# HeewoongNoh/DOSTransformer

Hardware: NVIDIA B200
Metric: train-step crystals/sec (fwd+bwd) (higher is better)
Workload: dtype bf16x3 operands, f32 accumulate

## Files before the change

dostransformer_b200/_lib.py:

```python
from __future__ import annotations

import ctypes as C
import os
from typing import Optional

import torch

_HERE = os.path.dirname(os.path.abspath(__file__))
LIB_PATH = os.environ.get("DOST_B200_LIB") or os.path.join(_HERE, "libdost_b200.so")

F32, F64 = 0, 1
ACT_NONE, ACT_RELU, ACT_LEAKY, ACT_PRELU = 0, 1, 2, 3
KC, MC = 0, 1
PREC_FMA, PREC_BF16X3, PREC_BF16 = 0, 1, 2
PRECISIONS = {"fp32": PREC_FMA, "bf16x3": PREC_BF16X3, "bf16": PREC_BF16}

_lib: Optional[C.CDLL] = None
ABI_VERSION = 15
DEVERR_MESSAGES = {1: "an index (edge_index / batch / system) is outside its table",
                   2: "a crystal has more atoms than the padding length given by the host (max_num_nodes)"}


class Seg(C.Structure):
    _fields_ = [("base", C.c_void_p), ("ld", C.c_longlong), ("idx", C.c_void_p), ("div", C.c_int),
# ... 36 lines not shown
        ("res_bstride", C.c_longlong),
        ("b_rowoff", C.c_void_p), ("c_rowoff", C.c_void_p), ("c_rowlim", C.c_void_p),
        ("colsum", C.c_void_p),
        ("out_gate", C.c_void_p), ("dact_gate", C.c_void_p), ("ld_gate", C.c_longlong),
    ]


_SIGNATURES = {
    "dost_abi_version": (C.c_int, []),
    "dost_last_error": (C.c_char_p, []),
    "dost_launch_count": (C.c_longlong, []),
    "dost_reset_launch_count": (None, []),
    "dost_device_errors_init": (C.c_int, []),
    "dost_device_errors": (C.c_uint, [C.c_int]),
    "dost_imax_scalar": (C.c_int, [C.c_void_p, C.c_int, C.c_void_p]),
    "dost_cast_i64_i32": (C.c_int, [C.c_void_p, C.c_void_p, C.c_longlong, C.c_void_p]),
    "dost_csr_workspace_bytes": (C.c_size_t, [C.c_longlong, C.c_longlong]),
    "dost_csr_build": (C.c_int, [C.c_void_p, C.c_longlong, C.c_longlong, C.c_void_p, C.c_void_p, C.c_void_p,
                                 C.c_void_p, C.c_size_t, C.c_void_p]),
    "dost_gemm_workspace_bytes": (C.c_size_t, [C.POINTER(Gemm)]),
    "dost_gemm": (C.c_int, [C.POINTER(Gemm), C.c_void_p, C.c_size_t, C.c_void_p]),
    "dost_gemm_bf16_workspace_bytes": (C.c_size_t, [C.POINTER(GemmBf16)]),
    "dost_gemm_bf16": (C.c_int, [C.POINTER(GemmBf16), C.c_void_p, C.c_size_t, C.c_void_p]),
    "dost_split_planes": (C.c_int, [C.c_void_p, C.c_longlong, C.c_longlong, C.c_int, C.c_void_p, C.c_void_p, C.c_longlong,
                                    C.c_void_p]),
    "dost_split_planes_multi": (C.c_int, [C.c_int, C.c_void_p, C.c_void_p, C.c_void_p, C.c_void_p, C.c_void_p, C.c_void_p,
                                          C.c_void_p, C.c_void_p]),
    "dost_split_planes_colsum_workspace_bytes": (C.c_size_t, [C.c_longlong, C.c_int, C.c_longlong]),
    "dost_split_planes_colsum": (C.c_int, [C.c_void_p, C.c_longlong, C.c_longlong, C.c_int, C.c_void_p, C.c_void_p, C.c_longlong,
                                           C.c_void_p, C.c_void_p, C.c_size_t, C.c_void_p]),
    "dost_ln_fwd_planes": (C.c_int, [C.c_void_p, C.c_longlong, C.c_void_p, C.c_void_p, C.c_void_p, C.c_void_p, C.c_longlong,
                                     C.c_void_p, C.c_void_p, C.c_void_p, C.c_void_p,
                                     C.c_void_p, C.c_void_p, C.c_longlong, C.c_void_p, C.c_longlong, C.c_int, C.c_void_p]),
    "dost_ln_bwd_planes_workspace_bytes": (C.c_size_t, [C.c_longlong, C.c_int]),
    "dost_ln_bwd_planes": (C.c_int, [C.c_void_p, C.c_longlong, C.c_void_p, C.c_longlong, C.c_void_p, C.c_void_p, C.c_void_p,
                                     C.c_void_p, C.c_void_p, C.c_longlong, C.c_void_p, C.c_void_p, C.c_void_p, C.c_longlong,
                                     C.c_void_p, C.c_void_p, C.c_void_p, C.c_void_p, C.c_longlong, C.c_int, C.c_void_p,
                                     C.c_size_t, C.c_void_p]),
    "dost_rowdot_fwd": (C.c_int, [C.c_void_p, C.c_longlong, C.c_void_p, C.c_void_p, C.c_void_p, C.c_longlong, C.c_int, C.c_void_p]),
    "dost_rowdot_bwd_workspace_bytes": (C.c_size_t, [C.c_longlong, C.c_int]),
    "dost_rowdot_bwd": (C.c_int, [C.c_void_p, C.c_void_p, C.c_longlong, C.c_void_p, C.c_void_p, C.c_void_p, C.c_longlong, C.c_int,
                                  C.c_void_p, C.c_size_t, C.c_void_p]),
    "dost_colsum_planes_workspace_bytes": (C.c_size_t, [C.c_longlong, C.c_int]),
    "dost_colsum_planes": (C.c_int, [C.c_void_p, C.c_void_p, C.c_longlong, C.c_longlong, C.c_int, C.c_void_p, C.c_void_p,
                                     C.c_size_t, C.c_void_p]),
    "dost_ln_fwd": (C.c_int, [C.c_int, C.c_void_p, C.c_longlong, C.c_void_p, C.c_void_p, C.c_void_p, C.c_void_p,
# ... 196 lines not shown
```

dostransformer_b200/csrc/gemm_bf.cu:

```cuda
#include <cuda.h>
#include <cuda_bf16.h>
#include <cstdlib>
#include "common.cuh"
#include "tc_ptx.cuh"

namespace dost {
namespace bf {

constexpr int BM = 128, BK = 64;
constexpr int kMaxStages = 6;
constexpr int kEpiBytes = 8 * 4096;
constexpr int kSmemBudget = 225 * 1024;

struct Maps {
  CUtensorMap a_hi[3], a_lo[3], b_hi, b_lo;
  CUtensorMap b_hi2, b_lo2;
  CUtensorMap c_out, c_hi, c_lo;
  CUtensorMap c_pre;
};

struct Params {
  int M, N, K;
  int a_nseg, a_kend[3];
  int a_mc, b_mc;
  int zmode, kchunk;
  long long c_bstride, res_bstride;
  const int* b_rowoff;
  const int* c_rowoff;
  const int* c_rowlim;
  int m_tiles, n_tiles, total_tiles;
  const float* bias;
  const float* rowbias; long long ld_rowbias; int rowbias_div;
  int act; float act_slope; const float* prelu_slope;
  float* out_pre; long long ld_pre;
  const __nv_bfloat16* dact_hi; long long ld_dact; float dact_slope;
  const float* residual; long long ld_res;
  float* out; long long ldc; int accumulate;
  __nv_bfloat16* out_hi; __nv_bfloat16* out_lo; long long ld_op;
  float* ws;
  float* colpart;
  unsigned int* out_gate;
  const unsigned int* dact_gate;
  long long ld_gate;
  int tma_epi;
};
// ... 48 lines not shown
  asm volatile("cp.async.bulk.tensor.2d.global.shared::cta.bulk_group [%0, {%1, %2}], [%3];" ::"l"(map), "r"(c0), "r"(c1), "r"(src)
               : "memory");
}

struct TileInfo {
  int m0, n0, kbeg, kend, nkt, z;
};
template <int BN, bool CTA2>
__device__ __forceinline__ TileInfo tile_info(const Params& p, int tile, int rank) {
  TileInfo t;
  const int per_z = p.m_tiles * p.n_tiles;
  t.z = tile / per_z;
  const int rem = tile - t.z * per_z;
  const int mt = rem / p.n_tiles, nt = rem - mt * p.n_tiles;
  t.m0 = mt * (CTA2 ? 2 * BM : BM) + rank * BM;
  t.n0 = nt * BN;
  t.kbeg = 0;
  t.kend = p.K;
  if (p.zmode == 2) {
    t.kbeg = t.z * p.kchunk;
    t.kend = min(p.K, t.kbeg + p.kchunk);
  }
  t.nkt = (t.kend > t.kbeg) ? (t.kend - t.kbeg + BK - 1) / BK : 0;
  return t;
}

template <int NSPLIT, int BN, bool CTA2, int EW = 8>
__global__ void __launch_bounds__((EW + 2) * 32, 1) gemm_bf_kernel(const __grid_constant__ Maps maps, const Params p) {
  constexpr int kEpiWarps = EW;
  constexpr bool SPLIT = NSPLIT == 3;
  constexpr int BNL = CTA2 ? BN / 2 : BN;
  constexpr int A_BYTES = BM * BK * 2, B_BYTES = BNL * BK * 2;
  constexpr int STAGE_BYTES = (SPLIT ? 2 : 1) * (A_BYTES + B_BYTES);
  constexpr int NSTAGE_RAW = (kSmemBudget - kEpiBytes) / STAGE_BYTES;
  constexpr int NSTAGE = NSTAGE_RAW < kMaxStages ? NSTAGE_RAW : kMaxStages;
  static_assert(NSTAGE >= 2, "need at least two smem stages");

  extern __shared__ __align__(1024) unsigned char smem_raw[];
  unsigned char* smem = reinterpret_cast<unsigned char*>((reinterpret_cast<uintptr_t>(smem_raw) + 1023) & ~uintptr_t(1023));
  float* epi_smem = reinterpret_cast<float*>(smem + NSTAGE * STAGE_BYTES);
  __shared__ __align__(8) unsigned long long bars[2 * kMaxStages + 4];
  __shared__ uint32_t tmem_base_s;

  const int warp = threadIdx.x >> 5, lane = threadIdx.x & 31;
  const uint32_t full0 = smem_u32(&bars[0]), empty0 = smem_u32(&bars[kMaxStages]);
  const uint32_t accf0 = smem_u32(&bars[2 * kMaxStages]), acce0 = smem_u32(&bars[2 * kMaxStages + 2]);
// ... 18 lines not shown
                   : "memory");
      asm volatile("tcgen05.relinquish_alloc_permit.cta_group::2.sync.aligned;" ::: "memory");
    } else {
      asm volatile("tcgen05.alloc.cta_group::1.sync.aligned.shared::cta.b32 [%0], %1;" ::"r"(smem_u32(&tmem_base_s)), "r"(512)
                   : "memory");
      asm volatile("tcgen05.relinquish_alloc_permit.cta_group::1.sync.aligned;" ::: "memory");
    }
  }
  tc_fence_before();
  __syncthreads();
  if (CTA2) cluster_sync_all();
  tc_fence_after();
  const uint32_t tmem_base = tmem_base_s;
  const bool a_mc = p.a_mc != 0, b_mc = p.b_mc != 0;

  if (warp == kEpiWarps + 1) {
    if (lane == 0) {
      int stage = 0;
      uint32_t phase = 0;
      for (int tile = tile0; tile < p.total_tiles; tile += tile_step) {
        const TileInfo t = tile_info<BN, CTA2>(p, tile, rank);
        const int nb0 = t.n0 + rank * BNL;
        int seg = 0;
        for (int kt = 0; kt < t.nkt; ++kt) {
          const int k0 = t.kbeg + kt * BK;
          while (seg + 1 < p.a_nseg && k0 >= p.a_kend[seg]) ++seg;
          const int kseg = k0 - (seg == 0 ? 0 : p.a_kend[seg - 1]);
          mbar_wait(empty0 + 8 * stage, phase ^ 1);
          const uint32_t bar = CTA2 ? mapa_rank(full0 + 8 * stage, 0) : full0 + 8 * stage;
          if (!CTA2) mbar_expect_tx(bar, STAGE_BYTES);
          else if (rank == 0) mbar_expect_tx(full0 + 8 * stage, 2 * STAGE_BYTES);
          const uint32_t sA = smem_u32(smem + stage * STAGE_BYTES);
          const uint32_t sB = sA + (SPLIT ? 2 : 1) * A_BYTES;
          const int zb = (p.zmode == 1) ? t.z : 0;
          auto load = [&](uint32_t dst, const CUtensorMap* m, int c0, int c1, int c2) {
            if (CTA2) tma_load_3d_2cta(dst, m, c0, c1, c2, bar);
            else tma_load_3d(dst, m, c0, c1, c2, bar);
          };
          const int brow = p.b_rowoff ? __ldg(p.b_rowoff + t.z) : 0;
          const int zbb = p.b_rowoff ? 0 : zb;
          if (!a_mc) {
            load(sA, &maps.a_hi[seg], kseg, t.m0, zb);
            if (SPLIT) load(sA + A_BYTES, &maps.a_lo[seg], kseg, t.m0, zb);
          } else {
#pragma unroll
            for (int b = 0; b < BM / 64; ++b) {
              load(sA + b * 8192, &maps.a_hi[0], t.m0 + 64 * b, k0, zb);
              if (SPLIT) load(sA + A_BYTES + b * 8192, &maps.a_lo[0], t.m0 + 64 * b, k0, zb);
            }
          }
          if (!b_mc) {
            load(sB, CTA2 ? &maps.b_hi2 : &maps.b_hi, k0, nb0 + brow, zbb);
            if (SPLIT) load(sB + B_BYTES, CTA2 ? &maps.b_lo2 : &maps.b_lo, k0, nb0 + brow, zbb);
          } else {
#pragma unroll
            for (int b = 0; b < BNL / 64; ++b) {
              load(sB + b * 8192, &maps.b_hi, nb0 + 64 * b, k0 + brow, zbb);
              if (SPLIT) load(sB + B_BYTES + b * 8192, &maps.b_lo, nb0 + 64 * b, k0 + brow, zbb);
            }
          }
          if (++stage == NSTAGE) {
            stage = 0;
            phase ^= 1;
          }
        }
      }
    }
  } else if (warp == kEpiWarps) {
    const uint32_t idesc = make_idesc(CTA2 ? 2 * BM : BM, BN, a_mc, b_mc);
    const uint32_t a_kstep = a_mc ? (2048 >> 4) : (32 >> 4);
    const uint32_t b_kstep = b_mc ? (2048 >> 4) : (32 >> 4);
    int stage = 0;
    uint32_t phase = 0;
    uint32_t acc_phase[2] = {0, 0};
    int local = 0;
    for (int tile = tile0; tile < p.total_tiles && rank == 0; tile += tile_step, ++local) {
      const TileInfo t = tile_info<BN, CTA2>(p, tile, rank);
      const int buf = local & 1;
      mbar_wait(acce0 + 8 * buf, acc_phase[buf] ^ 1);
      tc_fence_after();
      const uint32_t tmem_d = tmem_base + buf * BN;
// ... 746 lines not shown
  attr[0].val.clusterDim.x = 2;
  attr[0].val.clusterDim.y = 1;
  attr[0].val.clusterDim.z = 1;
  cfg.attrs = attr;
  cfg.numAttrs = 1;
  cudaError_t e = cudaLaunchKernelEx(&cfg, kern, maps, p);
  if (e != cudaSuccess) {
    set_error("gemm_bf16: cluster launch failed: %s", cudaGetErrorString(e));
    return DOST_ERR_LAUNCH;
  }
  return check_launch("gemm_bf16 (CTA pairs)");
}

static bool use_cta_pairs(int M, int N) {
  static const int enabled = [] {
    const char* e = getenv("DOST_GEMM_2CTA");
    return (e && e[0] == '0') ? 0 : 1;
  }();
  return enabled && M > 128 && N > 128;
}

static inline bool al16(const void* ptr) { return (reinterpret_cast<uintptr_t>(ptr) & 15) == 0; }

static int run(const dost_gemm_bf16_t* h, void* workspace, size_t workspace_bytes, cudaStream_t st) {
  DOST_REQUIRE(h->M > 0 && h->N > 0 && h->K > 0, "gemm_bf16: bad shape M=%d N=%d K=%d", h->M, h->N, h->K);
  DOST_REQUIRE(h->precision == DOST_PREC_BF16X3 || h->precision == DOST_PREC_BF16, "gemm_bf16: precision must be bf16x3 or bf16");
  DOST_REQUIRE(h->N % 4 == 0, "gemm_bf16: N must be a multiple of 4 (got %d)", h->N);
  const bool split3 = h->precision == DOST_PREC_BF16X3;
  const bool a_mc = h->a_mode == DOST_MC, b_mc = h->b_mode == DOST_MC;
  const int nseg = a_mc ? 1 : h->a_nseg;
  DOST_REQUIRE(nseg >= 1 && nseg <= 3, "gemm_bf16: a_nseg must be 1..3");
  const int bn = h->N <= 64 ? 64 : (h->N <= 128 ? 128 : 256);
  const bool pairs = use_cta_pairs(h->M, h->N);
  const int batch = h->batch < 1 ? 1 : h->batch;
  DOST_REQUIRE(!(batch > 1 && h->split_k > 1), "gemm_bf16: batch and split_k are exclusive");
  DOST_REQUIRE(batch == 1 || (h->a_nseg <= 1 && !h->rowbias && !h->out_pre && !h->dact_hi && !h->out_hi),
               "gemm_bf16: batched problems support bias / activation / residual / fp32 stores only");
  DOST_REQUIRE(batch == 1 || (h->a_bstride % 8 == 0 && h->b_bstride % 8 == 0 && h->c_bstride % 4 == 0 && h->res_bstride % 4 == 0),
               "gemm_bf16: batch strides must keep 16-byte alignment");

  Maps maps;
  Params p;
  p.M = h->M; p.N = h->N; p.K = h->K;
  p.a_nseg = nseg;
  p.a_mc = a_mc; p.b_mc = b_mc;
  int kacc = 0;
  for (int s = 0; s < nseg; ++s) {
// ... 35 lines not shown
        if (rc == DOST_OK && split3) rc = make_map(&maps.b_lo, pl.lo, h->K, pl.rows, pl.ld, bn);
        if (rc == DOST_OK && pairs) rc = make_map(&maps.b_hi2, pl.hi, h->K, pl.rows, pl.ld, 128);
        if (rc == DOST_OK && pairs && split3) rc = make_map(&maps.b_lo2, pl.lo, h->K, pl.rows, pl.ld, 128);
      } else {
        rc = make_map(&maps.b_hi, pl.hi, h->N, pl.rows, pl.ld, 64);
        if (rc == DOST_OK && split3) rc = make_map(&maps.b_lo, pl.lo, h->N, pl.rows, pl.ld, 64);
      }
    } else if (!b_mc) {
      const long long nrows = (pl.rows > 0 && pl.rows < h->N) ? pl.rows : h->N;
      rc = make_map(&maps.b_hi, pl.hi, h->K, nrows, pl.ld, bn, batch, h->b_bstride);
      if (rc == DOST_OK && split3) rc = make_map(&maps.b_lo, pl.lo, h->K, nrows, pl.ld, bn, batch, h->b_bstride);
      if (rc == DOST_OK && pairs) rc = make_map(&maps.b_hi2, pl.hi, h->K, nrows, pl.ld, 128, batch, h->b_bstride);
      if (rc == DOST_OK && pairs && split3) rc = make_map(&maps.b_lo2, pl.lo, h->K, nrows, pl.ld, 128, batch, h->b_bstride);
    } else {
      rc = make_map(&maps.b_hi, pl.hi, h->N, h->K, pl.ld, 64, batch, h->b_bstride);
      if (rc == DOST_OK && split3) rc = make_map(&maps.b_lo, pl.lo, h->N, h->K, pl.ld, 64, batch, h->b_bstride);
    }
    if (rc != DOST_OK) return rc;
    if (!split3) maps.b_lo = maps.b_hi;
    if (!pairs || b_mc) maps.b_hi2 = maps.b_hi;
    if (!pairs || b_mc || !split3) maps.b_lo2 = maps.b_hi2;
  }
  const int split = h->split_k < 1 ? 1 : h->split_k;
  p.zmode = split > 1 ? 2 : (batch > 1 ? 1 : 0);
  p.c_bstride = h->c_bstride;
  p.res_bstride = h->res_bstride;
  p.b_rowoff = h->b_rowoff;
  p.c_rowoff = h->c_rowoff;
  p.c_rowlim = h->c_rowlim;
  DOST_REQUIRE(!p.c_rowoff || p.c_rowlim, "gemm_bf16: ragged output needs both c_rowoff and c_rowlim");
  DOST_REQUIRE(split == 1 || !(p.b_rowoff || p.c_rowoff || p.c_rowlim), "gemm_bf16: ragged problems cannot be split along K");
  p.kchunk = 0;
  p.ws = nullptr;
  if (split > 1) {
    DOST_REQUIRE(!h->bias && !h->rowbias && h->act == DOST_ACT_NONE && !h->out_pre && !h->dact_hi && !h->residual && !h->out_hi,
                 "gemm_bf16: split_k supports only plain (accumulating) fp32 stores");
    const size_t need = sizeof(float) * (size_t)split * h->M * h->N;
    if (!workspace || workspace_bytes < need) {
      set_error("gemm_bf16: split_k workspace too small (%zu < %zu)", workspace_bytes, need);
      return DOST_ERR_WORKSPACE;
    }
    int kchunk = (h->K + split - 1) / split;
    p.kchunk = ((kchunk + BK - 1) / BK) * BK;
    p.ws = (float*)workspace;
  }
  p.m_tiles = pairs ? (h->M + 2 * BM - 1) / (2 * BM) : (h->M + BM - 1) / BM;
// ... 86 lines not shown
  }
  if (split > 1) {
    const long long total4 = (long long)h->M * h->N / 4;
    int blocks = (int)min64((total4 + 255) / 256, (long long)kNumSMs * 8);
    if (blocks < 1) blocks = 1;
    splitk_reduce_kernel<<<blocks, 256, 0, st>>>(p.ws, h->out, h->ldc, h->M, h->N, split, h->accumulate);
    rc = check_launch("gemm_bf16 split-k reduce");
  }
  return rc;
}

}
}

extern "C" size_t dost_gemm_bf16_workspace_bytes(const dost_gemm_bf16_t* g) {
  if (!g) return 0;
  if (g->colsum) return sizeof(float) * ((size_t)((g->M + 31) / 32) + dost::bf::kMidRows) * g->N;
  if (g->split_k <= 1) return 0;
  return sizeof(float) * (size_t)g->split_k * g->M * g->N;
}

extern "C" int dost_gemm_bf16(const dost_gemm_bf16_t* g, void* workspace, size_t workspace_bytes, dost_stream_t stream) {
  DOST_REQUIRE(g != nullptr, "gemm_bf16: null descriptor");
  return dost::bf::run(g, workspace, workspace_bytes, (cudaStream_t)stream);
}

extern "C" size_t dost_split_planes_colsum_workspace_bytes(long long rows, int cols, long long ldp) {
  return sizeof(float) * (size_t)dost::bf::split_colsum_chunks(rows, (int)ldp) * cols;
}

extern "C" int dost_split_planes_colsum(const float* x, long long ld, long long rows, int cols, void* hi, void* lo, long long ldp,
                                        float* colsum, void* workspace, size_t workspace_bytes, dost_stream_t stream) {
  DOST_REQUIRE(x && hi && colsum, "split_planes_colsum: null pointer");
  DOST_REQUIRE(rows > 0 && cols > 0 && ldp >= cols && ldp % 8 == 0, "split_planes_colsum: need rows > 0, ldp %% 8 == 0, ldp >= cols");
  DOST_REQUIRE(((uintptr_t)hi & 15) == 0 && ((uintptr_t)lo & 15) == 0, "split_planes_colsum: planes must be 16-byte aligned");
  const int nch = dost::bf::split_colsum_chunks(rows, (int)ldp);
  const size_t need = sizeof(float) * (size_t)nch * cols;
  if (!workspace || workspace_bytes < need) {
    dost::set_error("split_planes_colsum: workspace too small (%zu < %zu)", workspace_bytes, need);
    return DOST_ERR_WORKSPACE;
  }
  const int vec_ok = (((uintptr_t)x & 15) == 0 && ld % 4 == 0) ? 1 : 0;
  const long long rpc = (rows + nch - 1) / nch;
  dim3 grid((unsigned)((ldp / 8 + 31) / 32), nch);
  cudaStream_t st = (cudaStream_t)stream;
  dost::bf::split_planes_colsum_kernel<<<grid, 256, 0, st>>>(x, ld, rows, cols, (__nv_bfloat16*)hi, (__nv_bfloat16*)lo, (int)ldp, vec_ok,
                                                             rpc, (float*)workspace);
// ... 55 lines not shown
```

dostransformer_b200/ops.py:

```python
from __future__ import annotations

import ctypes as C
import math
from contextlib import nullcontext
import os
from dataclasses import dataclass, field
from typing import List, Optional, Sequence, Tuple

import torch

from . import _lib as L

NUM_SMS = 148

_PRECISION = L.PREC_FMA


def set_precision(name: str) -> None:
    global _PRECISION
    _PRECISION = L.PRECISIONS[name]


def get_precision() -> int:
    return _PRECISION
# ... 361 lines not shown
        cache[_planes_key(w)] = ((base._version, base.data_ptr(), _PLANES_GENERATION), Planes(hi, lo, w.shape[0], w.shape[1]))


def _planes_c(pl: Planes, width: int) -> L.PlanesC:
    c = L.PlanesC()
    c.hi = pl.hi.data_ptr()
    c.lo = pl.lo.data_ptr() if pl.lo is not None else None
    c.ld = pl.ld
    c.rows = pl.rows
    c.width = width
    return c


def gemm_planes(*, M: int, N: int, K: int, a: Sequence[Planes], a_mode: int, b: Planes, b_mode: int,
                out: Optional[torch.Tensor] = None, bias: Optional[torch.Tensor] = None,
                rowbias: Optional[torch.Tensor] = None, rowbias_div: int = 1, act: int = L.ACT_NONE, act_slope: float = 0.0,
                prelu_slope: Optional[torch.Tensor] = None, out_pre: Optional[torch.Tensor] = None,
                dact: Optional[Planes] = None, dact_slope: float = 0.0, residual: Optional[torch.Tensor] = None,
                accumulate: bool = False, split_k: int = 1, out_planes: Optional[Planes] = None,
                ldc: Optional[int] = None, prec: Optional[int] = None, batch: int = 1, a_bstride: int = 0, b_bstride: int = 0,
                c_bstride: int = 0, res_bstride: int = 0, ld_res: Optional[int] = None, b_rows: Optional[int] = None,
                b_rowoff: Optional[torch.Tensor] = None, c_rowoff: Optional[torch.Tensor] = None,
                c_rowlim: Optional[torch.Tensor] = None, colsum_out: Optional[torch.Tensor] = None,
                out_gate: Optional[torch.Tensor] = None, dact_gate: Optional[torch.Tensor] = None) -> None:
    g = L.GemmBf16()
    g.M, g.N, g.K = M, N, K
    g.a_mode, g.a_nseg = a_mode, len(a)
    for i, pl in enumerate(a):
        g.a[i] = _planes_c(pl, pl.cols if a_mode == L.KC else K)
    g.b_mode = b_mode
    g.b = _planes_c(b, 0)
    g.b.rows = b_rows if b_rows is not None else 0
    g.bias = bias.data_ptr() if bias is not None else None
    if rowbias is not None:
        g.rowbias, g.ld_rowbias, g.rowbias_div = rowbias.data_ptr(), _ld(rowbias), rowbias_div
    g.act, g.act_slope = act, act_slope
    g.prelu_slope = prelu_slope.data_ptr() if prelu_slope is not None else None
    if out_pre is not None:
        g.out_pre, g.ld_pre = out_pre.data_ptr(), _ld(out_pre)
    if dact is not None:
        g.dact_hi, g.ld_dact, g.dact_slope = dact.hi.data_ptr(), dact.ld, dact_slope
    if residual is not None:
        g.residual, g.ld_res = residual.data_ptr(), (ld_res if ld_res is not None else _ld(residual))
    if out is not None:
        g.out = out.data_ptr()
        g.ldc = ldc if ldc is not None else _ld(out)
    g.accumulate = 1 if accumulate else 0
    g.batch, g.a_bstride, g.b_bstride, g.c_bstride, g.res_bstride = batch, a_bstride, b_bstride, c_bstride, res_bstride
    g.b_rowoff = b_rowoff.data_ptr() if b_rowoff is not None else None
    g.c_rowoff = c_rowoff.data_ptr() if c_rowoff is not None else None
    g.c_rowlim = c_rowlim.data_ptr() if c_rowlim is not None else None
    if out_planes is not None:
        g.out_hi = out_planes.hi.data_ptr()
        g.out_lo = out_planes.lo.data_ptr() if out_planes.lo is not None else None
        g.ld_op = out_planes.ld
    g.split_k = split_k
    g.precision = _PRECISION if prec is None else prec
    g.colsum = colsum_out.data_ptr() if colsum_out is not None else None
    if out_gate is not None:
        g.out_gate, g.ld_gate = out_gate.data_ptr(), out_gate.stride(0)
    if dact_gate is not None:
        g.dact_gate, g.ld_gate, g.dact_slope = dact_gate.data_ptr(), dact_gate.stride(0), dact_slope
    lib = L.lib()
    ws, nb = None, 0
    if split_k > 1 or colsum_out is not None:
        nb = lib.dost_gemm_bf16_workspace_bytes(C.byref(g))
        ws = _ws(nb, b.hi.device)
    L.check(lib.dost_gemm_bf16(C.byref(g), L.p(ws), nb, L.stream()), "gemm_bf16")


def gate_bits_ok(M: int, N: int) -> bool:
    return M >= 32 and N % 32 == 0 and os.environ.get("DOST_GEMM_TMA_EPI", "1") != "0" and not L.switch("DOST_NO_FFN_GATE")


def tc_active(t: torch.Tensor) -> bool:
    return _PRECISION != L.PREC_FMA and t.dtype == torch.float32


def _with_lo() -> bool:
    return _PRECISION != L.PREC_BF16


def ln_fwd_planes(x2d: torch.Tensor, gamma, beta, slope=None, *, want_y: bool = False, want_planes: bool = True,
                  gather_add=None):
    M, W = x2d.shape
    ga = ia = gb = ib = None
    ldg = 0
    if gather_add is not None:
        ga, ia, gb, ib = gather_add
        ldg = _ld(ga)
        assert _ld(gb) == ldg
# ... 877 lines not shown
            dop = _grad_planes(d_out, S * T, H)
            d_out = d_out.contiguous()
            dP = torch.empty(S * T, npad, dtype=torch.float32, device=dev)
            gemm_planes(M=T, N=npad, K=H, a=[dop], a_mode=L.KC, b=kvp, b_mode=L.KC, b_rows=N + B, out=dP, batch=S,
                        a_bstride=T * dop.ld, c_bstride=T * npad, b_rowoff=ptr_ext)
            dsp = empty_planes(S * T, npad, dev, _with_lo())
            if ctx.fused and ctx.drop_p > 0:
                scores = torch.empty(S * T, npad, dtype=torch.float32, device=dev)
                gemm_planes(M=T, N=npad, K=H, a=[qp], a_mode=L.KC, b=kvp, b_mode=L.KC, b_rows=N + B, out=scores, batch=S,
                            a_bstride=T * qp.ld, c_bstride=T * npad, b_rowoff=ptr_ext)
            if ctx.fused and ctx.drop_p == 0:
                _ds_from_planes(pp, dP, S * T, npad, float(H) ** -0.5, dsp)
            else:
                L.check(lib.dost_xattn_softmax_bwd_dseed(L.p(scores), L.p(lse), L.p(dP), L.p(g.ptr), L.p(g.nmax), S * T, B, T, npad,
                                                         float(H) ** -0.5, L.p(dsp.hi), L.p(dsp.lo), dsp.ld, ctx.drop_p, ctx.seed,
                                                         L.p(ctx.seed_offset), L.stream()), "xattn_softmax_bwd")
            dq = torch.empty(S, T, H, dtype=torch.float32, device=dev)
            gemm_planes(M=T, N=H, K=npad, a=[dsp], a_mode=L.KC, b=kvp, b_mode=L.MC, b_rows=N + B, out=dq.view(S * T, H), batch=S,
                        a_bstride=T * dsp.ld, c_bstride=T * H, b_rowoff=ptr_ext)
            dkv = torch.empty(N, H, dtype=torch.float32, device=dev)
            dbrows = torch.empty(B, H, dtype=torch.float32, device=dev)
            if not L.switch("DOST_NO_XATTN_PADDED_DK"):
                dpad = torch.empty(S * npad, H, dtype=torch.float32, device=dev)
                gemm_planes(M=npad, N=H, K=T, a=[dsp], a_mode=L.MC, b=qp, b_mode=L.MC, out=dpad, batch=S, a_bstride=T * dsp.ld,
                            b_bstride=T * qp.ld, c_bstride=npad * H)
                gemm_planes(M=npad, N=H, K=T, a=[pp], a_mode=L.MC, b=dop, b_mode=L.MC, out=dpad, accumulate=True, batch=S,
                            a_bstride=T * pp.ld, b_bstride=T * dop.ld, c_bstride=npad * H)
                L.check(lib.dost_xattn_kv_pad_split(L.p(dpad), npad, reps, L.p(g.batch), L.p(g.ptr), N, B, H, L.p(dkv), L.p(dbrows),
                                                    L.stream()), "xattn_kv_pad_split")
                dph = colsum(dbrows)
                d_q = colsum(dq.view(S, T * H)).view(T, H) if ctx.bcast_q else dq
                d_resid = colsum(d_out.view(S, T * H)).view(T, H) if ctx.bcast_r else d_out
                return d_q, dkv, dph, d_resid, None, None, None, None, None, None, None
            dext = torch.empty(N + B, H, dtype=torch.float32, device=dev)
            p1, n1 = g.ragged(1)
            for rep in range(reps):
                r0, r1 = rep * B * T, (rep + 1) * B * T
                gemm_planes(M=npad, N=H, K=T, a=[_rows(dsp, r0, r1)], a_mode=L.MC, b=_rows(qp, r0, r1), b_mode=L.MC, out=dext,
                            accumulate=rep > 0, batch=B, a_bstride=T * dsp.ld, b_bstride=T * qp.ld, c_rowoff=p1, c_rowlim=n1)
                gemm_planes(M=npad, N=H, K=T, a=[_rows(pp, r0, r1)], a_mode=L.MC, b=_rows(dop, r0, r1), b_mode=L.MC, out=dext,
                            accumulate=True, batch=B, a_bstride=T * pp.ld, b_bstride=T * dop.ld, c_rowoff=p1, c_rowlim=n1)
            L.check(lib.dost_xattn_kv_ext_split(L.p(dext), L.p(g.batch), L.p(g.ptr), N, B, H, L.p(dkv), L.p(dbrows), L.stream()),
                    "xattn_kv_ext_split")
            dph = colsum(dbrows)
            d_q = colsum(dq.view(S, T * H)).view(T, H) if ctx.bcast_q else dq
            d_resid = colsum(d_out.view(S, T * H)).view(T, H) if ctx.bcast_r else d_out
        return d_q, dkv, dph, d_resid, None, None, None, None, None, None, None


def _maps_from_planes(pp: Planes, maps_out: torch.Tensor, rows: int, graph: Optional[CrystalGraph], T: int = 0, drop_p: float = 0.0,
# ... 24 lines not shown
                    maps_out=None):
    _check_seed_offset(seed_offset)
    H = kv.shape[1]
    _check_maps_out(maps_out, (S, q.shape[-2]), kv)
    if (tc_active(kv) and H % 128 == 0 and S % graph.B == 0 and graph.nmax_host is not None
            and graph.nkeys_host <= 1016 and q.shape[-2] >= 64 and not L.switch("DOST_NO_XATTN_TC")
            and (q.dim() == 3 or S == graph.B)):
        out = _CrossAttentionTC.apply(q, kv, phantom, resid, graph, _planes3(q), S, drop_p, seed, seed_offset, maps_out)
        out._dost_attn_out = True
        return out
    return _CrossAttention.apply(q, kv, phantom, resid, graph, S, drop_p, seed, seed_offset, maps_out)


class _SelfAttention(torch.autograd.Function):

    @staticmethod
    def forward(ctx, q, k, resid, drop_p: float, seed: int, seed_offset=None, maps_out=None):
        S, Lq, H = q.shape
        Lk = k.shape[1]
        qpl, kpl = _planes3(q), _planes3(k)
        q, k, resid = q.contiguous(), k.contiguous(), resid.contiguous()
        dev, dtype = q.device, q.dtype
        Lp = (Lk + 3) // 4 * 4
        ctx.on_planes = tc_active(q) and H % 8 == 0 and Lq * Lk * H >= (1 << 18) and not L.switch("DOST_NO_ATTNPLANES")
        if ctx.on_planes:
            qp = qpl if qpl is not None else split_planes(q.view(S * Lq, H))
            kp = kpl if kpl is not None else split_planes(k.view(S * Lk, H))
            ctx.drop_p, ctx.seed, ctx.seed_offset, ctx.prec = drop_p, seed, seed_offset, _PRECISION
            ctx.dims = (S, Lq, Lk, H, Lp)
            ctx.fused = fused_attention_ok(H, Lk, drop_p)
            if ctx.fused:
                out = torch.empty(S, Lq, H, dtype=dtype, device=dev)
                need = any(ctx.needs_input_grad[:3])
                pdp = empty_planes(S * Lq, Lk, dev, _with_lo()) if (need or maps_out is not None) else None
                _fused_attention_fwd(qp, kp, S * Lk, S, Lq, Lk, H, None, None, None, Lk, resid.view(S * Lq, H), Lq * H,
                                     out.view(S * Lq, H), pdp, drop_p, seed, seed_offset=seed_offset)
                if maps_out is not None:
                    _maps_from_planes(pdp, maps_out, S * Lq, None)
                if need:
                    ctx.save_for_backward(None, None, *_planes_save(qp), *_planes_save(kp), *_planes_save(pdp))
                return out
            scores = torch.empty(S, Lq, Lp, dtype=dtype, device=dev)
            gemm_planes(M=Lq, N=Lp, K=H, a=[qp], a_mode=L.KC, b=kp, b_mode=L.KC, b_rows=Lk, out=scores.view(S * Lq, Lp),
                        batch=S, a_bstride=Lq * qp.ld, b_bstride=Lk * kp.ld, c_bstride=Lq * Lp)
            pd = torch.empty_like(scores) if drop_p > 0 else scores
            pdp = empty_planes(S * Lq, Lk, dev, _with_lo())
# ... 62 lines not shown
    qp, kp = Planes(qh, ql, S * Lq, H), Planes(kh, kl, S * Lk, H)
    pdp = Planes(ph, pl_, S * Lq, Lk)
    dop = _grad_planes(d_out, S * Lq, H)
    d_out = d_out.contiguous()
    dpd = torch.empty(S, Lq, Lp, dtype=torch.float32, device=dev)
    gemm_planes(M=Lq, N=Lp, K=H, a=[dop], a_mode=L.KC, b=kp, b_mode=L.KC, b_rows=Lk, out=dpd.view(S * Lq, Lp), batch=S,
                a_bstride=Lq * dop.ld, b_bstride=Lk * kp.ld, c_bstride=Lq * Lp)
    dsp = empty_planes(S * Lq, Lk, dev, _with_lo())
    if ctx.fused and ctx.drop_p > 0:
        prob = torch.empty(S, Lq, Lp, dtype=torch.float32, device=dev)
        gemm_planes(M=Lq, N=Lp, K=H, a=[qp], a_mode=L.KC, b=kp, b_mode=L.KC, b_rows=Lk, out=prob.view(S * Lq, Lp), batch=S,
                    a_bstride=Lq * qp.ld, b_bstride=Lk * kp.ld, c_bstride=Lq * Lp)
        L.check(L.lib().dost_softmax_fwd(L.F32, L.p(prob), L.p(prob), None, S * Lq, Lk, Lp, scale, 0.0, 0, L.stream()), "softmax_fwd")
    if ctx.fused and ctx.drop_p == 0:
        _ds_from_planes(pdp, dpd.view(S * Lq, Lp), S * Lq, Lk, scale, dsp)
    else:
        L.check(L.lib().dost_softmax_bwd_planes_dseed(L.p(prob), L.p(dpd), None, S * Lq, Lk, Lp, scale, ctx.drop_p, ctx.seed,
                                                      L.p(ctx.seed_offset), L.p(dsp.hi), L.p(dsp.lo), dsp.ld, L.stream()),
                "softmax_bwd_planes")
    dq = torch.empty(S, Lq, H, dtype=torch.float32, device=dev)
    gemm_planes(M=Lq, N=H, K=Lk, a=[dsp], a_mode=L.KC, b=kp, b_mode=L.MC, out=dq.view(S * Lq, H), batch=S,
                a_bstride=Lq * dsp.ld, b_bstride=Lk * kp.ld, c_bstride=Lq * H)
    dk = torch.empty(S, Lk, H, dtype=torch.float32, device=dev)
    gemm_planes(M=Lk, N=H, K=Lq, a=[dsp], a_mode=L.MC, b=qp, b_mode=L.MC, out=dk.view(S * Lk, H), batch=S,
                a_bstride=Lq * dsp.ld, b_bstride=Lq * qp.ld, c_bstride=Lk * H)
    gemm_planes(M=Lk, N=H, K=Lq, a=[pdp], a_mode=L.MC, b=dop, b_mode=L.MC, out=dk.view(S * Lk, H), accumulate=True, batch=S,
                a_bstride=Lq * pdp.ld, b_bstride=Lq * dop.ld, c_bstride=Lk * H)
    return dq, dk, d_out, None, None, None, None


_SelfAttention._backward_planes = staticmethod(_self_attention_backward_planes)


def _cols(pl: Planes, cols: int) -> Planes:
    return Planes(pl.hi, pl.lo, pl.rows, cols)


def _planes3(t: torch.Tensor) -> Optional[Planes]:
    pl = getattr(t, "_dost_planes", None)
    if pl is not None and t.dim() == 3 and pl.rows == t.shape[0] * t.shape[1] and pl.cols == t.shape[2] and \
            (pl.lo is not None) == _with_lo():
        return pl
    return None


def self_attention(q, k, resid, drop_p: float = 0.0, seed: int = 0, seed_offset=None, maps_out=None):
# ... 98 lines not shown
```

include/dost.h:

```cpp
#ifndef DOST_H_
#define DOST_H_

#include <stddef.h>
#include <stdint.h>

#ifdef __cplusplus
extern "C" {
#endif

#define DOST_ABI_VERSION 15

enum { DOST_F32 = 0, DOST_F64 = 1 };
enum { DOST_OK = 0, DOST_ERR_ARG = -1, DOST_ERR_LAUNCH = -2, DOST_ERR_WORKSPACE = -3, DOST_ERR_UNSUPPORTED = -4 };
enum { DOST_ACT_NONE = 0, DOST_ACT_RELU = 1, DOST_ACT_LEAKY = 2, DOST_ACT_PRELU = 3 };
enum { DOST_PREC_FMA = 0, DOST_PREC_BF16X3 = 1 , DOST_PREC_BF16 = 2 };
enum { DOST_KC = 0 , DOST_MC = 1  };

typedef void* dost_stream_t;

int dost_abi_version(void);
const char* dost_last_error(void);
long long dost_launch_count(void);
void dost_reset_launch_count(void);

// ... 60 lines not shown
  const float* bias;
  const float* rowbias; long long ld_rowbias; int rowbias_div;
  int act; float act_slope; const float* prelu_slope;
  float* out_pre; long long ld_pre;
  const void* dact_hi; long long ld_dact; float dact_slope;
  const float* residual; long long ld_res;
  float* out; long long ldc; int accumulate;
  void* out_hi; void* out_lo; long long ld_op;
  int split_k;
  int precision;
  int batch;
  long long a_bstride, b_bstride, c_bstride, res_bstride;
  const int32_t* b_rowoff;
  const int32_t* c_rowoff;
  const int32_t* c_rowlim;
  float* colsum;
  uint32_t* out_gate;
  const uint32_t* dact_gate;
  long long ld_gate;
} dost_gemm_bf16_t;

size_t dost_gemm_bf16_workspace_bytes(const dost_gemm_bf16_t* g);
int dost_gemm_bf16(const dost_gemm_bf16_t* g, void* workspace, size_t workspace_bytes, dost_stream_t stream);
int dost_split_planes_multi(int ntensors, const float* const* x, const long long* ld, const long long* rows, const int* cols,
                            void* const* hi, void* const* lo, const long long* ldp, dost_stream_t stream);
int dost_split_planes(const float* x, long long ld, long long rows, int cols, void* hi, void* lo, long long ldp,
                      dost_stream_t stream);
size_t dost_split_planes_colsum_workspace_bytes(long long rows, int cols, long long ldp);
int dost_split_planes_colsum(const float* x, long long ld, long long rows, int cols, void* hi, void* lo, long long ldp,
                             float* colsum, void* workspace, size_t workspace_bytes, dost_stream_t stream);

int dost_ln_fwd_planes(float* x, long long ldx, const float* ga, const int32_t* ia, const float* gb, const int32_t* ib,
                       long long ldg, const float* gamma, const float* beta, const float* prelu_slope, float* y,
                       void* hi, void* lo, long long ldp, float* stats, long long M, int W, dost_stream_t stream);
size_t dost_ln_bwd_planes_workspace_bytes(long long M, int W);
int dost_ln_bwd_planes(const float* dy, long long ld_dy, const float* x, long long ldx, const float* stats,
                       const float* gamma, const float* beta, const float* prelu_slope, const float* dres,
                       long long ld_dres, float* dx, void* dx_hi, void* dx_lo, long long ldp, float* dgamma,
                       float* dbeta, float* dslope, float* dxsum, long long M, int W, void* workspace,
                       size_t workspace_bytes, dost_stream_t stream);
int dost_rowdot_fwd(const float* x, long long ldx, const float* w, const float* bias, float* out, long long M, int K,
                    dost_stream_t stream);
size_t dost_rowdot_bwd_workspace_bytes(long long M, int K);
int dost_rowdot_bwd(const float* dout, const float* x, long long ldx, const float* w, float* dx, float* dwb, long long M, int K,
                    void* workspace, size_t workspace_bytes, dost_stream_t stream);
size_t dost_colsum_planes_workspace_bytes(long long M, int W);
// ... 152 lines not shown
```

Before: 21100.

## Fuse paired attention-backward GEMMs into one kernel over concatenated K ranges

Adds a gemm_bf16_sum entry point that runs two GEMMs sharing an output tile as one K loop. The producer switches tensor maps to a second A/B pair once the first K range is done. The attention backward dK (and the cross-attention padded dK) now issues one launch instead of a GEMM plus an accumulate GEMM, so the output is read and written only once. When q is k, the dq term is folded in as a residual, which saves a further add. The risk is extra producer branching and more tensor map setup on the host.

```diff
diff --git a/dostransformer_b200/_lib.py b/dostransformer_b200/_lib.py
--- a/dostransformer_b200/_lib.py
+++ b/dostransformer_b200/_lib.py
@@ -82,6 +82,7 @@
     "dost_gemm": (C.c_int, [C.POINTER(Gemm), C.c_void_p, C.c_size_t, C.c_void_p]),
     "dost_gemm_bf16_workspace_bytes": (C.c_size_t, [C.POINTER(GemmBf16)]),
     "dost_gemm_bf16": (C.c_int, [C.POINTER(GemmBf16), C.c_void_p, C.c_size_t, C.c_void_p]),
+    "dost_gemm_bf16_sum": (C.c_int, [C.POINTER(GemmBf16), C.POINTER(GemmBf16), C.c_void_p, C.c_size_t, C.c_void_p]),
     "dost_split_planes": (C.c_int, [C.c_void_p, C.c_longlong, C.c_longlong, C.c_int, C.c_void_p, C.c_void_p, C.c_longlong,
                                     C.c_void_p]),
     "dost_split_planes_multi": (C.c_int, [C.c_int, C.c_void_p, C.c_void_p, C.c_void_p, C.c_void_p, C.c_void_p, C.c_void_p,
diff --git a/dostransformer_b200/csrc/gemm_bf.cu b/dostransformer_b200/csrc/gemm_bf.cu
--- a/dostransformer_b200/csrc/gemm_bf.cu
+++ b/dostransformer_b200/csrc/gemm_bf.cu
@@ -17,10 +17,12 @@
   CUtensorMap b_hi2, b_lo2;
   CUtensorMap c_out, c_hi, c_lo;
   CUtensorMap c_pre;
+  CUtensorMap a2_hi, a2_lo, b2_hi, b2_lo;
 };
 
 struct Params {
   int M, N, K;
+  int K2;
   int a_nseg, a_kend[3];
   int a_mc, b_mc;
   int zmode, kchunk;
@@ -115,6 +117,7 @@
     t.kend = min(p.K, t.kbeg + p.kchunk);
   }
   t.nkt = (t.kend > t.kbeg) ? (t.kend - t.kbeg + BK - 1) / BK : 0;
+  if (p.K2 > 0) t.nkt += (p.K2 + BK - 1) / BK;
   return t;
 }
 
@@ -179,10 +182,16 @@
         const TileInfo t = tile_info<BN, CTA2>(p, tile, rank);
         const int nb0 = t.n0 + rank * BNL;
         int seg = 0;
+        const int nkt1 = p.K2 > 0 ? (p.K + BK - 1) / BK : t.nkt;
         for (int kt = 0; kt < t.nkt; ++kt) {
-          const int k0 = t.kbeg + kt * BK;
+          const bool second = kt >= nkt1;
+          const int k0 = second ? (kt - nkt1) * BK : t.kbeg + kt * BK;
           while (seg + 1 < p.a_nseg && k0 >= p.a_kend[seg]) ++seg;
           const int kseg = k0 - (seg == 0 ? 0 : p.a_kend[seg - 1]);
+          const CUtensorMap* ma_hi = second ? &maps.a2_hi : &maps.a_hi[seg];
+          const CUtensorMap* ma_lo = second ? &maps.a2_lo : &maps.a_lo[seg];
+          const CUtensorMap* mb_hi = second ? &maps.b2_hi : ((CTA2 && !b_mc) ? &maps.b_hi2 : &maps.b_hi);
+          const CUtensorMap* mb_lo = second ? &maps.b2_lo : ((CTA2 && !b_mc) ? &maps.b_lo2 : &maps.b_lo);
           mbar_wait(empty0 + 8 * stage, phase ^ 1);
           const uint32_t bar = CTA2 ? mapa_rank(full0 + 8 * stage, 0) : full0 + 8 * stage;
           if (!CTA2) mbar_expect_tx(bar, STAGE_BYTES);
@@ -197,23 +206,23 @@
           const int brow = p.b_rowoff ? __ldg(p.b_rowoff + t.z) : 0;
           const int zbb = p.b_rowoff ? 0 : zb;
           if (!a_mc) {
-            load(sA, &maps.a_hi[seg], kseg, t.m0, zb);
-            if (SPLIT) load(sA + A_BYTES, &maps.a_lo[seg], kseg, t.m0, zb);
+            load(sA, ma_hi, kseg, t.m0, zb);
+            if (SPLIT) load(sA + A_BYTES, ma_lo, kseg, t.m0, zb);
           } else {
 #pragma unroll
             for (int b = 0; b < BM / 64; ++b) {
-              load(sA + b * 8192, &maps.a_hi[0], t.m0 + 64 * b, k0, zb);
-              if (SPLIT) load(sA + A_BYTES + b * 8192, &maps.a_lo[0], t.m0 + 64 * b, k0, zb);
+              load(sA + b * 8192, ma_hi, t.m0 + 64 * b, k0, zb);
+              if (SPLIT) load(sA + A_BYTES + b * 8192, ma_lo, t.m0 + 64 * b, k0, zb);
             }
           }
           if (!b_mc) {
-            load(sB, CTA2 ? &maps.b_hi2 : &maps.b_hi, k0, nb0 + brow, zbb);
-            if (SPLIT) load(sB + B_BYTES, CTA2 ? &maps.b_lo2 : &maps.b_lo, k0, nb0 + brow, zbb);
+            load(sB, mb_hi, k0, nb0 + brow, zbb);
+            if (SPLIT) load(sB + B_BYTES, mb_lo, k0, nb0 + brow, zbb);
           } else {
 #pragma unroll
             for (int b = 0; b < BNL / 64; ++b) {
-              load(sB + b * 8192, &maps.b_hi, nb0 + 64 * b, k0 + brow, zbb);
-              if (SPLIT) load(sB + B_BYTES + b * 8192, &maps.b_lo, nb0 + 64 * b, k0 + brow, zbb);
+              load(sB + b * 8192, mb_hi, nb0 + 64 * b, k0 + brow, zbb);
+              if (SPLIT) load(sB + B_BYTES + b * 8192, mb_lo, nb0 + 64 * b, k0 + brow, zbb);
             }
           }
           if (++stage == NSTAGE) {
@@ -1006,7 +1015,7 @@
 
 static inline bool al16(const void* ptr) { return (reinterpret_cast<uintptr_t>(ptr) & 15) == 0; }
 
-static int run(const dost_gemm_bf16_t* h, void* workspace, size_t workspace_bytes, cudaStream_t st) {
+static int run(const dost_gemm_bf16_t* h, const dost_gemm_bf16_t* h2, void* workspace, size_t workspace_bytes, cudaStream_t st) {
   DOST_REQUIRE(h->M > 0 && h->N > 0 && h->K > 0, "gemm_bf16: bad shape M=%d N=%d K=%d", h->M, h->N, h->K);
   DOST_REQUIRE(h->precision == DOST_PREC_BF16X3 || h->precision == DOST_PREC_BF16, "gemm_bf16: precision must be bf16x3 or bf16");
   DOST_REQUIRE(h->N % 4 == 0, "gemm_bf16: N must be a multiple of 4 (got %d)", h->N);
@@ -1088,6 +1097,40 @@
     if (!pairs || b_mc || !split3) maps.b_lo2 = maps.b_hi2;
   }
   const int split = h->split_k < 1 ? 1 : h->split_k;
+  p.K2 = 0;
+  maps.a2_hi = maps.a_hi[0];
+  maps.a2_lo = maps.a_lo[0];
+  maps.b2_hi = maps.b_hi2;
+  maps.b2_lo = maps.b_lo2;
+  if (h2) {
+    const dost_planes_t &a2 = h2->a[0], &b2 = h2->b;
+    DOST_REQUIRE(h2->K > 0 && nseg == 1 && split == 1 && !h->b_rowoff && !h->c_rowoff && !h->c_rowlim,
+                 "gemm_bf16_sum: needs K2 > 0, one A segment, no split_k and no ragged problems");
+    DOST_REQUIRE(a2.hi && (!split3 || a2.lo) && b2.hi && (!split3 || b2.lo), "gemm_bf16_sum: A2 / B2 planes missing");
+    DOST_REQUIRE(al16(a2.hi) && al16(a2.lo) && a2.ld % 8 == 0 && al16(b2.hi) && al16(b2.lo) && b2.ld % 8 == 0 &&
+                     (batch == 1 || (h2->a_bstride % 8 == 0 && h2->b_bstride % 8 == 0)),
+                 "gemm_bf16_sum: A2 / B2 planes must be 16-byte aligned, ld %% 8 == 0, batch strides %% 8 == 0");
+    const int K2 = h2->K;
+    p.K2 = K2;
+    int rc = a_mc ? make_map(&maps.a2_hi, a2.hi, h->M, K2, a2.ld, 64, batch, h2->a_bstride)
+                  : make_map(&maps.a2_hi, a2.hi, K2, batch > 1 ? h->M : a2.rows, a2.ld, BM, batch, h2->a_bstride);
+    if (rc == DOST_OK && split3)
+      rc = a_mc ? make_map(&maps.a2_lo, a2.lo, h->M, K2, a2.ld, 64, batch, h2->a_bstride)
+                : make_map(&maps.a2_lo, a2.lo, K2, batch > 1 ? h->M : a2.rows, a2.ld, BM, batch, h2->a_bstride);
+    const long long nrows2 = (b2.rows > 0 && b2.rows < h->N) ? b2.rows : h->N;
+    const int bbox = pairs ? 128 : bn;
+    if (rc == DOST_OK)
+      rc = b_mc ? make_map(&maps.b2_hi, b2.hi, h->N, K2, b2.ld, 64, batch, h2->b_bstride)
+                : make_map(&maps.b2_hi, b2.hi, K2, nrows2, b2.ld, bbox, batch, h2->b_bstride);
+    if (rc == DOST_OK && split3)
+      rc = b_mc ? make_map(&maps.b2_lo, b2.lo, h->N, K2, b2.ld, 64, batch, h2->b_bstride)
+                : make_map(&maps.b2_lo, b2.lo, K2, nrows2, b2.ld, bbox, batch, h2->b_bstride);
+    if (rc != DOST_OK) return rc;
+    if (!split3) {
+      maps.a2_lo = maps.a2_hi;
+      maps.b2_lo = maps.b2_hi;
+    }
+  }
   p.zmode = split > 1 ? 2 : (batch > 1 ? 1 : 0);
   p.c_bstride = h->c_bstride;
   p.res_bstride = h->res_bstride;
@@ -1220,7 +1263,13 @@
 
 extern "C" int dost_gemm_bf16(const dost_gemm_bf16_t* g, void* workspace, size_t workspace_bytes, dost_stream_t stream) {
   DOST_REQUIRE(g != nullptr, "gemm_bf16: null descriptor");
-  return dost::bf::run(g, workspace, workspace_bytes, (cudaStream_t)stream);
+  return dost::bf::run(g, nullptr, workspace, workspace_bytes, (cudaStream_t)stream);
+}
+
+extern "C" int dost_gemm_bf16_sum(const dost_gemm_bf16_t* g, const dost_gemm_bf16_t* g2, void* workspace, size_t workspace_bytes,
+                                  dost_stream_t stream) {
+  DOST_REQUIRE(g != nullptr && g2 != nullptr, "gemm_bf16_sum: null descriptor");
+  return dost::bf::run(g, g2, workspace, workspace_bytes, (cudaStream_t)stream);
 }
 
 extern "C" size_t dost_split_planes_colsum_workspace_bytes(long long rows, int cols, long long ldp) {
diff --git a/dostransformer_b200/ops.py b/dostransformer_b200/ops.py
--- a/dostransformer_b200/ops.py
+++ b/dostransformer_b200/ops.py
@@ -407,7 +407,9 @@
                 c_bstride: int = 0, res_bstride: int = 0, ld_res: Optional[int] = None, b_rows: Optional[int] = None,
                 b_rowoff: Optional[torch.Tensor] = None, c_rowoff: Optional[torch.Tensor] = None,
                 c_rowlim: Optional[torch.Tensor] = None, colsum_out: Optional[torch.Tensor] = None,
-                out_gate: Optional[torch.Tensor] = None, dact_gate: Optional[torch.Tensor] = None) -> None:
+                out_gate: Optional[torch.Tensor] = None, dact_gate: Optional[torch.Tensor] = None,
+                a2: Optional[Planes] = None, b2: Optional[Planes] = None, K2: int = 0, a2_bstride: int = 0,
+                b2_bstride: int = 0) -> None:
     g = L.GemmBf16()
     g.M, g.N, g.K = M, N, K
     g.a_mode, g.a_nseg = a_mode, len(a)
@@ -451,7 +453,14 @@
     if split_k > 1 or colsum_out is not None:
         nb = lib.dost_gemm_bf16_workspace_bytes(C.byref(g))
         ws = _ws(nb, b.hi.device)
-    L.check(lib.dost_gemm_bf16(C.byref(g), L.p(ws), nb, L.stream()), "gemm_bf16")
+    if a2 is None:
+        L.check(lib.dost_gemm_bf16(C.byref(g), L.p(ws), nb, L.stream()), "gemm_bf16")
+        return
+    g2 = L.GemmBf16()
+    g2.K, g2.a_bstride, g2.b_bstride = K2, a2_bstride, b2_bstride
+    g2.a[0] = _planes_c(a2, a2.cols if a_mode == L.KC else K2)
+    g2.b = _planes_c(b2, 0)
+    L.check(lib.dost_gemm_bf16_sum(C.byref(g), C.byref(g2), L.p(ws), nb, L.stream()), "gemm_bf16_sum")
 
 
 def gate_bits_ok(M: int, N: int) -> bool:
@@ -1375,10 +1384,15 @@
             dbrows = torch.empty(B, H, dtype=torch.float32, device=dev)
             if not L.switch("DOST_NO_XATTN_PADDED_DK"):
                 dpad = torch.empty(S * npad, H, dtype=torch.float32, device=dev)
-                gemm_planes(M=npad, N=H, K=T, a=[dsp], a_mode=L.MC, b=qp, b_mode=L.MC, out=dpad, batch=S, a_bstride=T * dsp.ld,
-                            b_bstride=T * qp.ld, c_bstride=npad * H)
-                gemm_planes(M=npad, N=H, K=T, a=[pp], a_mode=L.MC, b=dop, b_mode=L.MC, out=dpad, accumulate=True, batch=S,
-                            a_bstride=T * pp.ld, b_bstride=T * dop.ld, c_bstride=npad * H)
+                if not L.switch("DOST_NO_ATTN_FUSED_BWD"):
+                    gemm_planes(M=npad, N=H, K=T, a=[dsp], a_mode=L.MC, b=qp, b_mode=L.MC, out=dpad, batch=S,
+                                a_bstride=T * dsp.ld, b_bstride=T * qp.ld, c_bstride=npad * H,
+                                a2=pp, b2=dop, K2=T, a2_bstride=T * pp.ld, b2_bstride=T * dop.ld)
+                else:
+                    gemm_planes(M=npad, N=H, K=T, a=[dsp], a_mode=L.MC, b=qp, b_mode=L.MC, out=dpad, batch=S,
+                                a_bstride=T * dsp.ld, b_bstride=T * qp.ld, c_bstride=npad * H)
+                    gemm_planes(M=npad, N=H, K=T, a=[pp], a_mode=L.MC, b=dop, b_mode=L.MC, out=dpad, accumulate=True, batch=S,
+                                a_bstride=T * pp.ld, b_bstride=T * dop.ld, c_bstride=npad * H)
                 L.check(lib.dost_xattn_kv_pad_split(L.p(dpad), npad, reps, L.p(g.batch), L.p(g.ptr), N, B, H, L.p(dkv), L.p(dbrows),
                                                     L.stream()), "xattn_kv_pad_split")
                 dph = colsum(dbrows)
@@ -1449,6 +1463,7 @@
         q, k, resid = q.contiguous(), k.contiguous(), resid.contiguous()
         dev, dtype = q.device, q.dtype
         Lp = (Lk + 3) // 4 * 4
+        ctx.q_is_k = q is k
         ctx.on_planes = tc_active(q) and H % 8 == 0 and Lq * Lk * H >= (1 << 18) and not L.switch("DOST_NO_ATTNPLANES")
         if ctx.on_planes:
             qp = qpl if qpl is not None else split_planes(q.view(S * Lq, H))
@@ -1557,6 +1572,15 @@
     gemm_planes(M=Lq, N=H, K=Lk, a=[dsp], a_mode=L.KC, b=kp, b_mode=L.MC, out=dq.view(S * Lq, H), batch=S,
                 a_bstride=Lq * dsp.ld, b_bstride=Lk * kp.ld, c_bstride=Lq * H)
     dk = torch.empty(S, Lk, H, dtype=torch.float32, device=dev)
+    if not L.switch("DOST_NO_ATTN_FUSED_BWD"):
+        resid = dq.view(S * Lq, H) if ctx.q_is_k else None
+        gemm_planes(M=Lk, N=H, K=Lq, a=[dsp], a_mode=L.MC, b=qp, b_mode=L.MC, out=dk.view(S * Lk, H), batch=S,
+                    a_bstride=Lq * dsp.ld, b_bstride=Lq * qp.ld, c_bstride=Lk * H,
+                    residual=resid, res_bstride=Lq * H if ctx.q_is_k else 0,
+                    a2=pdp, b2=dop, K2=Lq, a2_bstride=Lq * pdp.ld, b2_bstride=Lq * dop.ld)
+        if ctx.q_is_k:
+            return dk, None, d_out, None, None, None, None
+        return dq, dk, d_out, None, None, None, None
     gemm_planes(M=Lk, N=H, K=Lq, a=[dsp], a_mode=L.MC, b=qp, b_mode=L.MC, out=dk.view(S * Lk, H), batch=S,
                 a_bstride=Lq * dsp.ld, b_bstride=Lq * qp.ld, c_bstride=Lk * H)
     gemm_planes(M=Lk, N=H, K=Lq, a=[pdp], a_mode=L.MC, b=dop, b_mode=L.MC, out=dk.view(S * Lk, H), accumulate=True, batch=S,
diff --git a/include/dost.h b/include/dost.h
--- a/include/dost.h
+++ b/include/dost.h
@@ -106,6 +106,8 @@
 
 size_t dost_gemm_bf16_workspace_bytes(const dost_gemm_bf16_t* g);
 int dost_gemm_bf16(const dost_gemm_bf16_t* g, void* workspace, size_t workspace_bytes, dost_stream_t stream);
+int dost_gemm_bf16_sum(const dost_gemm_bf16_t* g, const dost_gemm_bf16_t* g2, void* workspace, size_t workspace_bytes,
+                       dost_stream_t stream);
 int dost_split_planes_multi(int ntensors, const float* const* x, const long long* ld, const long long* rows, const int* cols,
                             void* const* hi, void* const* lo, const long long* ldp, dost_stream_t stream);
 int dost_split_planes(const float* x, long long ld, long long rows, int cols, void* hi, void* lo, long long ldp,
```

New measurement: 21260, median of 6. No clear change (+0.8%).
